# skeskinen/bert.cpp

Measured on AMD Instinct MI355X. Metric: sentences/sec (seq_len=128), higher is better.
Workload: dtype f16; 1 GPU; all-MiniLM-L6-v2 f16, batch=256 seq_len=128; per_gpu_batch=256, global_batch=256, seq_len=128, weights=f16, parallelism=dp1 (replicated weights, sharded sentences)

## Files before the change

### bert.cpp_amd/csrc/layer_tail.hip

```cpp
#include "tile_stream.h"

namespace bert_hip {

namespace {

constexpr int LT_TILE = 16384;
#ifndef LT_ABLATE
#define LT_ABLATE 0
#endif
#ifndef LT_UPRIO
#define LT_UPRIO 1
#endif
#ifndef LT_GELU_BATCH
#define LT_GELU_BATCH 0
#endif
#ifndef LT_DMA_SPLIT
#define LT_DMA_SPLIT 1
#endif
#ifndef LT_DPRIO
#define LT_DPRIO 0
#endif

typedef float f32x2 __attribute__((ext_vector_type(2)));

// ... 46 lines not shown
    asm volatile("ds_read_b64 %0, %1 offset:%2" : "=v"(v) : "v"(addr), "n"(OFF) : "memory");
    return v;
}
template <int OFF>
__device__ __forceinline__ f32x4 lds_read_f32x4_h(unsigned addr) {
    f32x4 v;
    asm volatile("ds_read_b128 %0, %1 offset:%2" : "=v"(v) : "v"(addr), "n"(OFF) : "memory");
    return v;
}
template <int OFF>
__device__ __forceinline__ f16x8 frag_read(unsigned addr) {
    if (LT_ABLATE & 4) { f16x8 z = (f16x8)(_Float16)0.f; asm volatile("" : "+v"(z) : "v"(addr)); return z; }
    return lds_read_b128_u<OFF>(addr);
}

__device__ __forceinline__ void dma_m0(unsigned lds) {
    if (LT_ABLATE & 1) return;
    asm volatile("s_mov_b32 m0, %0" : : "s"(lds) : "memory");
}
template <int PIECE>
__device__ __forceinline__ void dma_piece(const char *gbase, unsigned voff) {
    if (LT_ABLATE & 1) return;
    asm volatile("global_load_lds_dwordx4 %0, %1 offset:%2" : : "v"(voff), "s"(gbase - PIECE * 1024), "n"(PIECE * 1024) : "memory");
}

__device__ __forceinline__ f32x16 mfma16(const f16x8 &a, const f16x8 &b, const f32x16 &c) {
    if (LT_ABLATE & 8) { f32x16 r = c; asm volatile("" : "+v"(r[0]) : "v"(a), "v"(b)); return r; }
    return __builtin_amdgcn_mfma_f32_32x32x16_f16(a, b, c, 0, 0, 0);
}

}

template <int NT, int WT, bool RAGGED = false>
__device__ __forceinline__ void layer_tail_body(const TailArgs &a, char *smem, const int tok0, const int rows, const int tid) {
    constexpr bool Q4 = WT != GW_F16;
    constexpr int VMQ = Q4 ? 63 : 0;
    constexpr int H = 128 * NT, NBH = 2 * NT, NB = 4 * NT, NQ = 8 * NT, NYH = 4 * NT;
    constexpr int P = NT * NT;
    constexpr int NG = NT;
    constexpr int LAGT = NT + NG;
    const int I = a.I, NC = I / 64;
    const int lane = tid & 63;
    const int wave = __builtin_amdgcn_readfirstlane(tid >> 6);
    const int t = wave & 3, role = wave >> 2;
    const int l31 = lane & 31, hi = lane >> 5;
    const int tok_w = tok0 + t * 32;
    const int row_l = RAGGED ? tok0 + min(t * 32 + l31, rows - 1) : tok_w + l31;

    char *ringU = smem;
    char *ringD = smem + 3 * LT_TILE;
    char *G = smem + 6 * LT_TILE;
    float *ST = (float *)(G + 32768);
    float *cbo = ST + 8 * 64;
    float *cg1 = cbo + H, *cbe1 = cg1 + H, *cb2 = cbe1 + H, *cg2 = cb2 + H, *cbe2 = cg2 + H, *cb1 = cbe2 + H;

    {
        constexpr int NPB = 4;
        const float *const src[6] = {a.bo, a.g1, a.be1, a.b2, a.g2, a.be2};
        float pv[6];
        f32x4 bq[NPB];
#pragma unroll
        for (int k = 0; k < 6; ++k) pv[k] = tid < H ? src[k][tid] : 0.f;
#pragma unroll
        for (int k = 0; k < NPB; ++k) {
            const int i4 = (k * 512 + tid) * 4;
            bq[k] = i4 < I ? *(const f32x4 *)(a.b1 + i4) : f32x4{0.f, 0.f, 0.f, 0.f};
        }
// ... 87 lines not shown
    auto dma_proj = [&](int n3, int kt, unsigned tile) __attribute__((always_inline)) {
        if constexpr (Q4) q4_request_rows(a.wo_qs, a.wo_sc, n3 * (H / 64) + kt);
        else dma128(wo + (size_t)n3 * 128 * H + kt * 64, offH, H * 2, tile);
    };
    auto dma_up = [&](int c, int j, unsigned offU, unsigned tile) __attribute__((always_inline)) {
        if constexpr (Q4) q4_request_up(c, j);
        else dma_up_f16(c, j, offU, tile);
    };

    const unsigned aR = lds_addr(ringU) + (unsigned)off64(l31, hi);
    const unsigned aUp = lds_addr(ringU) + (unsigned)(l31 * 256 + ((hi ^ (l31 & 15)) << 4));

    int slot = 0;
    [[maybe_unused]] int tl = 1;
    [[maybe_unused]] const bool tlU = tid == 0, tlD = tid == 256;
    LT_STAMP(tlU, 0);
    auto pre_close = [&]() __attribute__((always_inline)) { LT_STAMP_FINE(tlU, 128 + tl); LT_STAMP_FINE(tlD, 256 + tl); };
    auto next_slot = [&]() __attribute__((always_inline)) { slot = slot == 2 ? 0 : slot + 1; LT_STAMP(tlU, tl); ++tl; };
    auto slot_plus2 = [&]() __attribute__((always_inline)) { return slot == 0 ? 2 : slot - 1; };
    [[maybe_unused]] auto slot_plus1 = [&]() __attribute__((always_inline)) { return slot == 2 ? 0 : slot + 1; };
    using PLAIN = std::false_type; using PERMUTED = std::true_type;

    auto proj_request = [&](int p, int s) __attribute__((always_inline)) {
        const int n3 = p / NT, q = p % NT;
        if (role == 0) dma_proj(n3, 2 * q, ldsU + s * LT_TILE);
        else dma_proj(n3, 2 * q + 1, ldsD + s * LT_TILE);
    };
    proj_request(0, 0);
    q4_expand_rows(PLAIN{}, role ? ringD : ringU);
    proj_request(1, 1);
    LT_STAMP(tlU, 384);
    asm volatile("s_waitcnt vmcnt(0) lgkmcnt(0)\n\ts_barrier" ::: "memory");
    LT_STAMP(tlU, 385);
#pragma unroll
    for (int b = 0; b < NBH; ++b)
#pragma unroll
        for (int gq = 0; gq < 4; ++gq) {
            const f32x4 bv = *(const f32x4 *)(cbo + (b >> 1) * 128 + role * 64 + (b & 1) * 32 + 8 * gq + 4 * hi);
#pragma unroll
            for (int e = 0; e < 4; ++e) accp[b][4 * gq + e] = (float)xv[b][gq][e] + bv[e];
        }
#pragma unroll
    for (int b = 0; b < NBH; ++b) asm volatile("" : "+v"(accp[b]));
    __builtin_amdgcn_s_waitcnt(0xc07f);
    static_for<P>([&](auto p_tag) __attribute__((always_inline)) {
        constexpr int p = decltype(p_tag)::value, n3 = p / NT, q = p % NT, p2 = p + 2;
        const unsigned bA = aR + (unsigned)(slot * LT_TILE + role * 8192), bB = bA + 3 * LT_TILE;
        f16x8 Fa[4], Fb[4];
        auto rd = [&](unsigned base, int g2, f16x8 (&F)[4]) __attribute__((always_inline)) {
            const unsigned a0 = base ^ (unsigned)((2 * g2) << 5), a1 = base ^ (unsigned)((2 * g2 + 1) << 5);
            F[0] = frag_read<0>(a0); F[1] = frag_read<4096>(a0);
            F[2] = frag_read<0>(a1); F[3] = frag_read<4096>(a1);
        };
        auto mm = [&](f16x8 (&F)[4], int ks) __attribute__((always_inline)) {
            accp[n3 * 2 + 0] = mfma16(F[0], bf[ks], accp[n3 * 2 + 0]);
            accp[n3 * 2 + 1] = mfma16(F[1], bf[ks], accp[n3 * 2 + 1]);
            accp[n3 * 2 + 0] = mfma16(F[2], bf[ks + 1], accp[n3 * 2 + 0]);
            accp[n3 * 2 + 1] = mfma16(F[3], bf[ks + 1], accp[n3 * 2 + 1]);
        };
        auto q4_turn = [&]() __attribute__((always_inline)) {
            if constexpr (p + 1 < P) q4_expand_rows(PLAIN{}, (role ? ringD : ringU) + slot_plus1() * LT_TILE);
            else if (role == 1) q4_expand_up(ringU + slot_plus1() * LT_TILE);
            const int s2 = slot_plus2();
            if constexpr (p2 < P) proj_request(p2, s2);
            else if (role == 1) dma_up(0, p2 - P, up_offset(), ldsU + s2 * LT_TILE);
        };
// ... 362 lines not shown
                    request(std::integral_constant<bool, up>{}, FF{}, c * NT + d + LAGT + 2, 0);
                    if constexpr (pend_dn) q4_expand_rows(PERMUTED{}, ringD + slot_plus1() * LT_TILE);
                    request(FF{}, std::integral_constant<bool, dn>{}, 0, c * NT + d + 2);
                    __builtin_amdgcn_sched_barrier(0);
                }
                rd(std::integral_constant<int, 0>{}, Fa, ga);
                rd(std::integral_constant<int, 1>{}, Fb, gb);
                wait_group(N5{}, Fa, ga);
                mm(Fa, ga);
                rd(std::integral_constant<int, 2>{}, Fa, ga);
                if constexpr (!Q4) {
                    if constexpr (LT_DMA_SPLIT) request(std::integral_constant<bool, up>{}, FF{}, c * NT + d + LAGT + 2, 0);
                    else request(std::integral_constant<bool, up>{}, std::integral_constant<bool, dn>{}, c * NT + d + LAGT + 2, c * NT + d + 2);
                }
                wait_group(N5{}, Fb, gb);
                mm(Fb, gb);
                rd(std::integral_constant<int, 3>{}, Fb, gb);
                if constexpr (!Q4 && LT_DMA_SPLIT) request(FF{}, std::integral_constant<bool, dn>{}, 0, c * NT + d + 2);
                wait_group(N5{}, Fa, ga);
                mm(Fa, ga);
                wait_group(N0{}, Fb, gb);
                mm(Fb, gb);
                pre_close();
                close_interval<Q4 ? 63 : (up ? 4 : 0) + (dn ? 4 : 0)>();
                next_slot();
            });
        };
        static_assert(LAGT == 2 * NT, "the request schedule below assumes D runs two chunks behind");
        (void)NUP;
        for (int c = 0; c + 3 < NC; ++c) d_chunk(std::integral_constant<int, NT>{}, FF{}, TT{}, c);
        d_chunk(std::integral_constant<int, NT - 2>{}, FF{}, TT{}, NC - 3);
        d_chunk(std::integral_constant<int, 0>{}, FF{}, FF{}, NC - 2);
        d_chunk(std::integral_constant<int, 0>{}, TT{}, FF{}, NC - 1);

        {
            char *S = smem + t * (64 * H);
            int lane = (int)__builtin_amdgcn_mbcnt_hi(~0u, __builtin_amdgcn_mbcnt_lo(~0u, 0u));
            asm volatile("" : "+v"(lane));
            const int hi = lane >> 5;
            {
                const char *const xu = ringU + t * (NYH * 1024) + lane * 16;
#pragma unroll
                for (int n3 = 0; n3 < NT; ++n3) {
                    f16x8 yu[4];
#pragma unroll
                    for (int m = 0; m < 4; ++m) yu[m] = *(const f16x8 *)(xu + (4 * n3 + m) * 1024);
#pragma unroll
                    for (int m = 0; m < 4; ++m)
#pragma unroll
                        for (int e = 0; e < 8; ++e) acc2[4 * n3 + (m >> 1)][8 * (m & 1) + e] += (float)yu[m][e];
                    asm volatile("" ::: "memory");
                }
            }
            asm volatile("s_waitcnt lgkmcnt(0)\n\ts_barrier" ::: "memory");
            float s1 = 0.f, s2 = 0.f;
#pragma unroll
            for (int n = 0; n < NB; ++n)
#pragma unroll
                for (int r = 0; r < 16; ++r) { s1 += acc2[n][r]; s2 = __builtin_fmaf(acc2[n][r], acc2[n][r], s2); }
            s1 += __shfl_xor(s1, 32);
            s2 += __shfl_xor(s2, 32);
            float rstd, nmr;
            layernorm_scale(s1, s2, 1.0f / H, rstd, nmr);
#pragma unroll
            for (int n = 0; n < NB; ++n) {
                f32x4 gv[4], bv[4];
// ... 94 lines not shown
```

### bert.cpp_amd/csrc/model_kernel.hip

```cpp
#define BERT_HIP_PHASES_ONLY
#include "qkv_attention2.hip"
#include "layer_tail.hip"
#undef BERT_HIP_PHASES_ONLY
#include "pool_normalize.h"

namespace bert_hip {

#ifdef BERT_HIP_MODEL_TIMELINE
static __device__ unsigned long long g_tl_model[1024 * 32];
#define MK_STAMP(i) do { const int mk_i = (i); if (threadIdx.x == 0 && mk_i < 32) g_tl_model[(blockIdx.x & 1023) * 32 + mk_i] = __builtin_amdgcn_s_memrealtime(); } while (0)
#else
#define MK_STAMP(i) do { } while (0)
#endif

namespace {

constexpr int MODEL_MAX_LAYERS = 12;

struct ModelLayerArgs {
    const half_t *wqkv, *wo, *w1p, *w2p;
    const float *bqkv, *bo, *g1, *be1, *b1, *b2, *g2, *be2;
};
struct ModelArgs {
    half_t *x, *ctx;
    const int32_t *cu;
    const int2 *groups;
    const int *n_groups;
    int n_layer, n_head, n_sent, I, slot_mask;
    float *pooled;
    int *status;
    int max_len;
    ModelLayerArgs layer[MODEL_MAX_LAYERS];
};

}

template <int NT, bool RAGGED>
__global__ __launch_bounds__(512, 2) void model_kernel(ModelArgs m) {
    extern __shared__ __attribute__((aligned(16))) char smem[];
    const int window = (int)blockIdx.x;
    int tok0 = window * 128, rows = 128, first = window, count = 1;
    if constexpr (RAGGED) {
        if (m.groups) {
            if (m.n_groups && window >= *m.n_groups) return;
            const int2 g = m.groups[window];
            first = g.x; count = g.y;
        }
        if (count <= 0 || first >= m.n_sent) return;
        tok0 = m.cu[first];
        rows = min(m.cu[first + count] - tok0, 128);
    }
    const int wave_index = __builtin_amdgcn_readfirstlane((int)threadIdx.x >> 6);
    auto thread_id = [&]() __attribute__((always_inline)) {
        int ln = (int)__builtin_amdgcn_mbcnt_hi(~0u, __builtin_amdgcn_mbcnt_lo(~0u, 0u)), w = wave_index;
        asm volatile("" : "+v"(ln), "+s"(w));
        return w * 64 + ln;
    };
    MK_STAMP(0);
    const int n_layer = rows > 0 ? m.n_layer : 0;
    for (int l = 0; l < n_layer; ++l) {
        const ModelLayerArgs &L = m.layer[l];
        int tid = thread_id();
        {
            Qkv2Args q;
            q.x = m.x; q.w = L.wqkv; q.qs = nullptr; q.sc = nullptr; q.bias = L.bqkv; q.cu = m.cu; q.groups = RAGGED ? m.groups : nullptr; q.n_groups = nullptr;
            q.out = m.ctx; q.n_head = m.n_head; q.n_sent = m.n_sent; q.spw = 1; q.slot_mask = m.slot_mask;
            qkv_attention2_body<2 * NT, NT, GW_F16>(q, smem, window, tid);
        }
        __builtin_amdgcn_fence(__ATOMIC_RELEASE, "workgroup");
        asm volatile("s_waitcnt vmcnt(0) lgkmcnt(0)\n\ts_barrier" ::: "memory");
        __builtin_amdgcn_fence(__ATOMIC_ACQUIRE, "workgroup");
        MK_STAMP(1 + 2 * l);
        tid = thread_id();
        {
            TailArgs t;
            t.ctx = m.ctx; t.x = m.x; t.wo = L.wo; t.w1p = L.w1p; t.w2p = L.w2p;
            t.wo_qs = t.w1_qs = t.w2_qs = nullptr; t.wo_sc = t.w1_sc = t.w2_sc = nullptr;
            t.bo = L.bo; t.g1 = L.g1; t.be1 = L.be1; t.b1 = L.b1; t.b2 = L.b2; t.g2 = L.g2; t.be2 = L.be2; t.out = m.x; t.I = m.I;
            layer_tail_body<NT, GW_F16, RAGGED>(t, smem, tok0, rows, tid);
        }
        __builtin_amdgcn_fence(__ATOMIC_RELEASE, "workgroup");
        asm volatile("s_waitcnt vmcnt(0) lgkmcnt(0)\n\ts_barrier" ::: "memory");
        __builtin_amdgcn_fence(__ATOMIC_ACQUIRE, "workgroup");
        MK_STAMP(2 + 2 * l);
    }
    if (m.pooled) {
        const int tid = thread_id();
        for (int j = 0; j < count; ++j) {
            const int b = first + j, t0 = m.cu[b];
            int n = m.cu[b + 1] - t0;
            if (!RAGGED && (t0 != tok0 || n != 128)) n = -1;
            pool_normalize_sentence(m.x, t0, n, b, 128 * NT, m.max_len, m.status, m.pooled, (float *)smem, tid, tid < 256);
            __syncthreads();
        }
    }
    MK_STAMP(1 + 2 * n_layer);
}

bool model_kernel_supported(const GemmWeight &Wqkv, const GemmWeight &Wo, const GemmWeight &W1, const GemmWeight &W2, int n_layer,
                            int n_head, int d_head, int max_len) {
    const int H = n_head * d_head;
    return n_layer <= MODEL_MAX_LAYERS && (H == 256 || H == 384) && max_len >= 1 && max_len <= 128 &&
           Wqkv.type == GW_F16 && Wo.type == GW_F16 && qkv_attention2_supported(Wqkv, n_head, d_head, max_len) && layer_tail_supported(Wo, W1, W2);
}

void launch_model_kernel(const ModelLayerWeights *layers, int n_layer, half_t *x, half_t *ctx, const int32_t *cu_seqlens, int n_sentences,
                         int n_tokens, const int2 *groups, int n_groups, const int *n_groups_dev, int n_head, float *pooled, int max_len,
                         int *status, int slots, hipStream_t stream) {
    ModelArgs m;
    m.pooled = pooled; m.status = status; m.max_len = max_len;
    m.x = x; m.ctx = ctx; m.cu = cu_seqlens; m.groups = groups; m.n_groups = n_groups_dev;
    m.n_layer = n_layer; m.n_head = n_head; m.n_sent = n_sentences; m.I = layers[0].W1->N; m.slot_mask = slots - 1;
    for (int l = 0; l < n_layer; ++l) {
        const ModelLayerWeights &s = layers[l];
        ModelLayerArgs &d = m.layer[l];
        d.wqkv = s.Wqkv->w16; d.wo = s.Wo->w16; d.w1p = s.W1->w16p; d.w2p = s.W2->w16p;
        d.bqkv = s.bqkv; d.bo = s.bo; d.g1 = s.g1; d.be1 = s.be1; d.b1 = s.b1; d.b2 = s.b2; d.g2 = s.g2; d.be2 = s.be2;
    }
    const int H = layers[0].W1->K, KT = H / 64, GB = KT / 2;
    const size_t lds_q = (size_t)3 * GB * Q2_TILE + 2 * (2 * Q2_WIN * 64 + 32 * Q2_VT_LD * 2) + (size_t)2 * H * sizeof(float);
    const size_t lds = std::max(lds_q, layer_tail_lds(H, m.I));
    const bool full = (long long)n_sentences * 128 == n_tokens;
    const int grid = full || !groups ? n_sentences : n_groups;
    static DeviceFlags configured[4];
    auto go = [&](auto kernel, int which) {
        configure_once(configured[which], [&] { (void)hipFuncSetAttribute((const void *)kernel, hipFuncAttributeMaxDynamicSharedMemorySize, 160 * 1024); });
        BERT_LAUNCH(kernel, dim3(grid), dim3(512), lds, stream, m);
#ifdef BERT_HIP_MODEL_TIMELINE
        static int shots = 0;
        if (grid >= 256 && shots++ == 30) {
            (void)hipDeviceSynchronize();
            static unsigned long long h[1024 * 32];
            (void)hipMemcpyFromSymbol(h, HIP_SYMBOL(g_tl_model), sizeof(h));
            const int nw = grid < 1024 ? grid : 1024, ns = 2 + 2 * n_layer;
            unsigned long long t0 = ~0ull;
            for (int w = 0; w < nw; ++w) t0 = h[w * 32] < t0 ? h[w * 32] : t0;
            fprintf(stderr, "model_kernel timeline, %d workgroups (us after the first workgroup's start: min mean max):\n", nw);
            for (int i = 0; i < ns; ++i) {
                double lo = 1e30, hi = 0, sum = 0;
                for (int w = 0; w < nw; ++w) { const double v = (double)(h[w * 32 + i] - t0) * 0.01; lo = v < lo ? v : lo; hi = v > hi ? v : hi; sum += v; }
                fprintf(stderr, "  stamp %2d: %8.2f %8.2f %8.2f\n", i, lo, sum / nw, hi);
            }
            fprintf(stderr, "  mean phase durations (window, tail) per layer:");
            for (int l = 0; l < n_layer; ++l) {
                double a = 0, b = 0;
                for (int w = 0; w < nw; ++w) { a += (double)(h[w * 32 + 1 + 2 * l] - h[w * 32 + 2 * l]) * 0.01; b += (double)(h[w * 32 + 2 + 2 * l] - h[w * 32 + 1 + 2 * l]) * 0.01; }
                fprintf(stderr, " (%.1f, %.1f)", a / nw, b / nw);
            }
            fprintf(stderr, "\n  mean end per XCD:");
            for (int x = 0; x < 8; ++x) {
                double e = 0; int c = 0;
                for (int w = x; w < nw; w += 8) { e += (double)(h[w * 32 + ns - 1] - t0) * 0.01; ++c; }
                fprintf(stderr, " %.1f", e / c);
            }
            fprintf(stderr, "\n  mean end per eighth of the grid:");
            for (int x = 0; x < 8; ++x) {
                double e = 0; int c = 0;
                for (int w = x * nw / 8; w < (x + 1) * nw / 8; ++w) { e += (double)(h[w * 32 + ns - 1] - t0) * 0.01; ++c; }
                fprintf(stderr, " %.1f", e / c);
            }
            double pl = 0;
            for (int w = 0; w < nw; ++w) pl += (double)(h[w * 32 + 1 + 2 * n_layer] - h[w * 32 + 2 * n_layer]) * 0.01;
            fprintf(stderr, "; pooling %.2f\n", pl / nw);
        }
#endif
    };
    if (full) { if (H == 256) go(model_kernel<2, false>, 0); else go(model_kernel<3, false>, 1); }
    else { if (H == 256) go(model_kernel<2, true>, 2); else go(model_kernel<3, true>, 3); }
}

}
```

### bert.cpp_amd/csrc/qkv_attention2.hip

```cpp
#include "tile_stream.h"

#ifndef Q2_PM
#define Q2_PM 3
#endif
#ifndef Q2_PRIO
#define Q2_PRIO 0
#endif

namespace bert_hip {

namespace {

constexpr int Q2_WIN = 128;
constexpr int Q2_TILE = 12288;
constexpr int Q2_VT_LD = Q2_WIN + 4;

struct Qkv2Args {
    const half_t *x;
    const half_t *w;
    const uint4 *qs;
    const void *sc;
    const float *bias;
    const int32_t *cu;
    const int2 *groups;
// ... 15 lines not shown
__device__ __forceinline__ void q2_wait6(f16x8 (&f)[2][3]) {
    asm volatile("s_waitcnt lgkmcnt(6)"
                 : "+v"(f[0][0]), "+v"(f[0][1]), "+v"(f[0][2]), "+v"(f[1][0]), "+v"(f[1][1]), "+v"(f[1][2]) : : "memory");
}
template <int VM>
__device__ __forceinline__ void q2_slab_barrier(f16x8 (&f)[2][3]) {
    asm volatile("s_waitcnt vmcnt(%6) lgkmcnt(0)\n\ts_barrier"
                 : "+v"(f[0][0]), "+v"(f[0][1]), "+v"(f[0][2]), "+v"(f[1][0]), "+v"(f[1][1]), "+v"(f[1][2]) : "n"(VM) : "memory");
}
__device__ __forceinline__ void q2_wait14(f16x8 (&f)[2][3]) {
    asm volatile("s_waitcnt lgkmcnt(14)"
                 : "+v"(f[0][0]), "+v"(f[0][1]), "+v"(f[0][2]), "+v"(f[1][0]), "+v"(f[1][1]), "+v"(f[1][2]) : : "memory");
}
__device__ __forceinline__ void q2_wait0_bias(f16x8 (&f)[2][3], f32x4 (&bq)[4], f32x4 (&bk)[4]) {
    asm volatile("s_waitcnt lgkmcnt(0)"
                 : "+v"(f[0][0]), "+v"(f[0][1]), "+v"(f[0][2]), "+v"(f[1][0]), "+v"(f[1][1]), "+v"(f[1][2]),
                   "+v"(bq[0]), "+v"(bq[1]), "+v"(bq[2]), "+v"(bq[3]), "+v"(bk[0]), "+v"(bk[1]), "+v"(bk[2]), "+v"(bk[3]) : : "memory");
}
template <int OFF>
__device__ __forceinline__ f32x4 q2_read_f32x4(unsigned addr) {
    f32x4 v;
    asm volatile("ds_read_b128 %0, %1 offset:%2" : "=v"(v) : "v"(addr), "n"(OFF));
    return v;
}
__device__ __forceinline__ void q2_take(float &bv) { asm volatile("" : "+v"(bv)); }
template <int VM>
__device__ __forceinline__ void q2_head_barrier() {
    asm volatile("s_waitcnt vmcnt(%0) lgkmcnt(0)\n\ts_barrier" : : "n"(VM) : "memory");
}

}

template <int KT, int GB, int WT>
__device__ __forceinline__ void qkv_attention2_body(const Qkv2Args &a, char *smem, const int window, const int tid) {
    constexpr bool Q4 = WT != GW_F16;
    constexpr int H = 64 * KT, NBAR = KT / GB, SLAB = GB * Q2_TILE, PPS = 3 * GB;
    static_assert(KT == 2 * GB && NBAR == 2, "");
    constexpr int QKV_BYTES = 2 * Q2_WIN * 64 + 32 * Q2_VT_LD * 2;
    char *RING = smem;
    char *QKV = smem + 3 * SLAB;
    float *BS = (float *)(QKV + 2 * QKV_BYTES);

    const int lane = tid & 63;
    const int wave = __builtin_amdgcn_readfirstlane(tid >> 6);
    const int l31 = lane & 31, hi = lane >> 5;
    const int blk = wave & 3;
    const int n_head = a.n_head;
    TL_STAMP_AT(tid == 256, 120);
    TL_REALTIME_AT(tid == 256, 121);
    TL_STAMP_AT(tid == 0, 250);
    TL_REALTIME_AT(tid == 0, 251);

    const int wp = blk;
    const unsigned loff = (unsigned)(((wp * 8 + (lane >> 3)) * H + (((lane & 7) ^ (((wp & 1) << 2) | ((lane >> 4) & 3))) * 8)) * 2);
    auto dma_piece = [&](const char *hbase, auto j_tag, int dslot, auto i_tag) __attribute__((always_inline)) {
        constexpr int i = decltype(i_tag)::value, j = decltype(j_tag)::value, t = i / 3, rb = i % 3;
        const char *src = hbase + ((size_t)rb * H * H + (size_t)(j * GB + t) * 64) * 2;
        __builtin_amdgcn_global_load_lds(AS_GLOBAL(src + loff), AS_LDS(RING + dslot * SLAB + t * Q2_TILE + rb * 4096 + wp * 1024), 16, 0, 0);
    };
    const char *const wbase = (const char *)a.w;
    if constexpr (!Q4) {
        if (wave >= 4) static_for<PPS>([&](auto i) __attribute__((always_inline)) { dma_piece(wbase, std::integral_constant<int, 0>{}, 0, i); });
    }

    int first, count;
    if (a.groups) {
        if (a.n_groups && window >= *a.n_groups) {
            asm volatile("s_waitcnt vmcnt(0)" ::: "memory");
            return;
        }
        const int2 g = a.groups[window];
        first = g.x; count = g.y;
    }
    else { first = window * a.spw; count = min(a.spw, a.n_sent - first); }
    if (count <= 0) {
        asm volatile("s_waitcnt vmcnt(0)" ::: "memory");
        return;
    }
    const int slot = blk * 32 + l31;
    int gtok = -1, k0 = 0, k1 = 0;
    {
        const int place = a.groups ? 128 : 128 / a.spw;
        int off = 0;
        for (int j = 0; j < count; ++j) {
            const int t0 = a.cu[first + j], n = min(a.cu[first + j + 1] - t0, place);
            if (slot >= off && slot < off + n) { gtok = t0 + slot - off; k0 = off; k1 = off + n; }
            off = (off + n + a.slot_mask) & ~a.slot_mask;
        }
    }

    if (wave >= 4) {
        f16x8 bf[4 * KT];
        {
            const int gt = gtok >= 0 ? gtok : a.cu[first];
            const half_t *xr = a.x + (size_t)gt * H + 8 * hi;
#pragma unroll
            for (int ks = 0; ks < 4 * KT; ++ks) asm volatile("global_load_dwordx4 %0, %1, off" : "=v"(bf[ks]) : "v"(xr + 16 * ks));
        }
        if constexpr (!Q4) static_for<PPS>([&](auto i) __attribute__((always_inline)) { dma_piece(wbase, std::integral_constant<int, NBAR - 1>{}, 1, i); });

        constexpr int NRAW = GB;
        [[maybe_unused]] RawBlock raw[NRAW];
        auto q4_image_of_lane = [&]() __attribute__((always_inline)) {
            int ln = (int)__builtin_amdgcn_mbcnt_hi(~0u, __builtin_amdgcn_mbcnt_lo(~0u, 0u));
            asm volatile("" : "+v"(ln));
            return (ln >> 1) * 128 + (((4 * (ln & 1)) ^ ((ln >> 2) & 7)) << 4);
        };
        auto q4_rb = [&](int hq, int j, int i) __attribute__((always_inline)) { return (blk + i + 2 * hq + j) & 3; };
        auto q4_request = [&](int hq, int j, int i) __attribute__((always_inline)) {
            if constexpr (Q4) {
                const int rb = q4_rb(hq, j, i);
                if (rb == 3) return;
                const int sbase = ((rb * (H / 128) + (hq >> 2)) * (H / 64) + j * GB + i) * 256 + (hq & 3) * 64;
                raw[i] = q4_load_block<WT>(a.qs + sbase, WT == GW_Q4_0 ? (const void *)((const unsigned short *)a.sc + sbase) : (const void *)((const unsigned *)a.sc + sbase), (size_t)lane);
            }
        };
        auto q4_expand = [&](int hq, int j, int dslot, int i) __attribute__((always_inline)) {
            if constexpr (Q4) {
                const int rb = q4_rb(hq, j, i);
                if (rb == 3) return;
                char *const base = RING + dslot * SLAB + i * Q2_TILE + rb * 4096;
                const int q4_image = q4_image_of_lane();
                q4_expand_block<WT, false>(raw[i], [&](int k) __attribute__((always_inline)) { return base + (q4_image ^ (k << 4)); });
            }
        };
        if constexpr (Q4) {
            RawBlock first[2][NRAW];
#pragma unroll
            for (int j = 0; j < 2; ++j)
#pragma unroll
// ... 8 lines not shown
                    raw[i] = first[j][i];
                    q4_expand(0, j, j, i);
                }
        }
        const unsigned aX0 = lds_addr(RING) + off64(l31, hi);
        unsigned aS[4];
        int rslot = 0;
        auto set_slot = [&]() __attribute__((always_inline)) {
#pragma unroll
            for (int kk = 0; kk < 4; ++kk) aS[kk] = (aX0 ^ (unsigned)(kk << 5)) + (unsigned)rslot * SLAB;
        };
        set_slot();
        f16x8 F[2][2][3];
        f32x16 acc[3];
        auto read_half = [&](auto par_tag, auto tt_tag, auto half_tag) __attribute__((always_inline)) {
            constexpr int par = decltype(par_tag)::value, tt = decltype(tt_tag)::value, half = decltype(half_tag)::value;
#pragma unroll
            for (int i = 0; i < 2; ++i) {
                F[par][i][0] = q2_read_b128<tt * Q2_TILE>(aS[2 * half + i]);
                F[par][i][1] = q2_read_b128<tt * Q2_TILE + 4096>(aS[2 * half + i]);
                F[par][i][2] = q2_read_b128<tt * Q2_TILE + 8192>(aS[2 * half + i]);
            }
        };
        [[maybe_unused]] const bool tl_sel = tid == 256;
        TL_STAMP_AT(tl_sel, 0);
        asm volatile("s_waitcnt vmcnt(%0) lgkmcnt(0)\n\ts_barrier" : : "n"(Q4 ? 0 : PPS) : "memory");
#pragma unroll
        for (int ks = 0; ks < 4 * KT; ++ks) asm volatile("" : "+v"(bf[ks]));
        if constexpr (Q4) {
#pragma unroll
            for (int i = 0; i < NRAW; ++i) q4_request(min(1, n_head - 1), 0, i);
        }
        TL_STAMP_AT(tl_sel, 1);
        read_half(std::integral_constant<int, 0>{}, std::integral_constant<int, 0>{}, std::integral_constant<int, 0>{});

        const unsigned aBias = lds_addr(BS) + 16 * hi;
        for (int h = 0; h < n_head; ++h) {
            char *QS = QKV + (h & 1) * QKV_BYTES, *KS = QS + Q2_WIN * 64;
            half_t *VT = (half_t *)(KS + Q2_WIN * 64);
            float bv;
            if constexpr (Q4) bv = a.bias[2 * H + h * 32 + l31];
            else asm volatile("global_load_dword %0, %1, off" : "=v"(bv) : "v"(a.bias + 2 * H + h * 32 + l31));
            f32x4 bq[4], bk[4];
            const char *const hnext = wbase + (size_t)min(h + 1, n_head - 1) * 32 * H * 2;
#pragma unroll
            for (int m = 0; m < 3; ++m)
#pragma unroll
                for (int r = 0; r < 16; ++r) acc[m][r] = 0.f;
            constexpr int LT0 = 2 * KT - 2, LT1 = 2 * KT - 1;
            auto pieces = [&](auto hh_tag, auto m_tag) __attribute__((always_inline)) {
                constexpr int hh = decltype(hh_tag)::value, m = decltype(m_tag)::value, hs = hh % (2 * GB);
                constexpr int i0 = (3 * hs + 1) / 2, i1 = (3 * (hs + 1) + 1) / 2;
                const int dslot = (hh == 2 * GB - 1) ? (rslot == 2 ? 0 : rslot + 1) : (rslot == 0 ? 2 : rslot - 1);
                if constexpr (Q4) {
                    constexpr int j = (hh >> 1) / GB;
                    if constexpr (m == 1) {
                        if constexpr (hs < GB) { if (h + 1 < n_head) q4_expand(h + 1, j, dslot, hs); }
                        else q4_request(min(j == 0 ? h + 1 : h + 2, n_head - 1), j ^ 1, hs - GB);
                    }
                } else {
                if constexpr (m == 1) dma_piece(hnext, std::integral_constant<int, (hh >> 1) / GB>{}, dslot, std::integral_constant<int, i0>{});
                if constexpr (m == 4 && i1 - i0 == 2) dma_piece(hnext, std::integral_constant<int, (hh >> 1) / GB>{}, dslot, std::integral_constant<int, i0 + 1>{});
                }
            };
            auto mma = [&](auto par_tag, auto i_tag, auto rb_tag, auto ks_tag) __attribute__((always_inline)) {
                constexpr int par = decltype(par_tag)::value, i = decltype(i_tag)::value, rb = decltype(rb_tag)::value, ks = decltype(ks_tag)::value;
// ... 54 lines not shown
                    }
#pragma unroll
                    for (int gg = 0; gg < 4; ++gg) {
                        f16x4 ov;
#pragma unroll
                        for (int e = 0; e < 4; ++e) ov[e] = (_Float16)(acc[2][4 * gg + e] + bv);
                        *(f16x4 *)(VT + l31 * Q2_VT_LD + blk * 32 + 8 * gg + 4 * hi) = ov;
                    }
                }
            });
            if (h < 8) TL_STAMP_AT(tl_sel, 2 + 6 * h + 4);
            q2_head_barrier<Q4 ? 63 : PPS>();
            if (h < 8) TL_STAMP_AT(tl_sel, 2 + 6 * h + 5);
            rslot = rslot == 2 ? 0 : rslot + 1;
            set_slot();
            read_half(std::integral_constant<int, 0>{}, std::integral_constant<int, 0>{}, std::integral_constant<int, 0>{});
        }
        TL_STAMP_AT(tl_sel, 60);
        asm volatile("s_waitcnt vmcnt(0)" ::: "memory");
    } else {
        unsigned need = 0, inner = 0;
#pragma unroll
        for (int kt = 0; kt < 4; ++kt) {
            const bool nd = gtok >= 0 && k0 < 32 * kt + 32 && k1 > 32 * kt;
            const bool in = gtok < 0 || (k0 <= 32 * kt && k1 >= 32 * kt + 32);
            if (__any(nd)) need |= 1u << kt;
            if (__all(in)) inner |= 1u << kt;
        }
        need = __builtin_amdgcn_readfirstlane(need);
        inner = __builtin_amdgcn_readfirstlane(inner);
        const unsigned klen = (unsigned)(k1 - k0);
        const int kbase = 4 * hi - k0;
        const float sc = 1.44269504088896340736f / __builtin_sqrtf(32.0f);
        for (int i = tid; i < 2 * H; i += 256) BS[i] = a.bias[i];
        asm volatile("s_waitcnt vmcnt(0) lgkmcnt(0)\n\ts_barrier" ::: "memory");

        if constexpr (Q2_PRIO > 0) __builtin_amdgcn_s_setprio(Q2_PRIO);
        [[maybe_unused]] const bool tl_sel = tid == 0;
        auto attend = [&](int hh, auto wb_tag, auto fast_tag, int tb) __attribute__((always_inline)) {
            constexpr bool WB = decltype(wb_tag)::value, FAST = decltype(fast_tag)::value;
            const char *QS = QKV + (hh & 1) * QKV_BYTES, *KS = QS + Q2_WIN * 64;
            const half_t *VT = (const half_t *)(KS + Q2_WIN * 64);
            f32x16 s[4];
            f16x8 qf[2];
#pragma unroll
            for (int kk = 0; kk < 2; ++kk) qf[kk] = *(const f16x8 *)(QS + q2_off32(slot, kk * 2 + hi));
            float mx = -INFINITY;
            int kb = kbase;
            unsigned kl = klen;
            if constexpr (!FAST) asm volatile("" : "+v"(kb), "+v"(kl));
#pragma unroll
            for (int kt = 0; kt < 4; ++kt) {
                if (FAST || (need & (1u << kt))) {
#pragma unroll
                    for (int r = 0; r < 16; ++r) s[kt][r] = 0.f;
#pragma unroll
                    for (int kk = 0; kk < 2; ++kk) {
                        const f16x8 kf = *(const f16x8 *)(KS + q2_off32(kt * 32 + l31, kk * 2 + hi));
                        s[kt] = __builtin_amdgcn_mfma_f32_32x32x16_f16(kf, qf[kk], s[kt], 0, 0, 0);
                    }
                    if (FAST || (inner & (1u << kt))) {
#pragma unroll
                        for (int r = 0; r < 16; ++r) mx = fmaxf(mx, s[kt][r]);
                    } else {
#pragma unroll
                        for (int r = 0; r < 16; ++r) {
                            const bool ok = (unsigned)(kt * 32 + (r & 3) + 8 * (r >> 2) + kb) < kl;
                            const float v = ok ? s[kt][r] : -INFINITY;
// ... 24 lines not shown
                        const f16x8 pf = softmax_p8(s[kt][8 * st], s[kt][8 * st + 1], s[kt][8 * st + 2], s[kt][8 * st + 3], s[kt][8 * st + 4],
                                                    s[kt][8 * st + 5], s[kt][8 * st + 6], s[kt][8 * st + 7], sc, mx, psum);
                        const int key0 = kt * 32 + 16 * st + 4 * hi;
                        const half_t *vr = VT + l31 * Q2_VT_LD + key0;
                        const f16x4 v0 = *(const f16x4 *)vr, v1 = *(const f16x4 *)(vr + 8);
                        f16x8 vf;
#pragma unroll
                        for (int e = 0; e < 4; ++e) { vf[e] = v0[e]; vf[4 + e] = v1[e]; }
                        o = __builtin_amdgcn_mfma_f32_32x32x16_f16(vf, pf, o, 0, 0, 0);
                    }
                }
                if constexpr (WB) {
                    if (kt + 4 == Q2_PM) {
                        if (tb < 8) TL_STAMP_AT(tl_sel, 128 + 6 * tb + 1);
                        asm volatile("s_barrier" ::: "memory");
                        if (tb < 8) TL_STAMP_AT(tl_sel, 128 + 6 * tb + 2);
                    }
                }
            }
            psum = xor32_sum(psum);
            if (gtok >= 0) {
                const float inv = 1.0f / psum;
                half_t *op = a.out + (size_t)gtok * H + hh * 32;
#pragma unroll
                for (int gq = 0; gq < 4; ++gq) {
                    f16x4 ov;
#pragma unroll
                    for (int e = 0; e < 4; ++e) ov[e] = (_Float16)rounded_f32(o[4 * gq + e] * inv);
                    *(f16x4 *)(op + 8 * gq + 4 * hi) = ov;
                }
            }
        };
        const bool fast = need == 0xFu && inner == 0xFu;
        asm volatile("s_barrier" ::: "memory");
        asm volatile("s_barrier" ::: "memory");
        for (int h = 1; h < n_head; ++h) {
            if (h < 8) TL_STAMP_AT(tl_sel, 128 + 6 * h);
            if (fast) attend(h - 1, std::true_type{}, std::true_type{}, h);
            else attend(h - 1, std::true_type{}, std::false_type{}, h);
            if (h < 8) TL_STAMP_AT(tl_sel, 128 + 6 * h + 5);
            asm volatile("s_barrier" ::: "memory");
        }
        TL_STAMP_AT(tl_sel, 190);
        if (fast) attend(n_head - 1, std::false_type{}, std::true_type{}, 0);
        else attend(n_head - 1, std::false_type{}, std::false_type{}, 0);
        TL_STAMP_AT(tl_sel, 192);
        TL_STAMP_AT(tl_sel, 252);
        TL_REALTIME_AT(tl_sel, 253);
    }
}

template <int KT, int GB, int WT>
__global__ __launch_bounds__(512, 2) void qkv_attention2_kernel(Qkv2Args a) {
    extern __shared__ __attribute__((aligned(16))) char smem[];
    qkv_attention2_body<KT, GB, WT>(a, smem, (int)blockIdx.x, (int)threadIdx.x);
}

#ifndef BERT_HIP_PHASES_ONLY
constexpr int BW_THREADS = 512;

template <int SLOT>
__global__ __launch_bounds__(BW_THREADS) void build_windows_kernel(const int32_t *__restrict__ cu, int B, int2 *__restrict__ windows,
                                                                   int *__restrict__ n_windows) {
    constexpr int BW_STATES = 128 / SLOT + 1;
    __shared__ unsigned char exit_state[BW_THREADS][BW_STATES];
    __shared__ int closes[BW_THREADS][BW_STATES];
    __shared__ int opened[BW_THREADS][BW_STATES];
    __shared__ int entry_fill[BW_THREADS], entry_first[BW_THREADS], entry_index[BW_THREADS];
    const int t = threadIdx.x, per = (B + BW_THREADS - 1) / BW_THREADS, n_blocks = per ? (B + per - 1) / per : 0;
    const int b0 = min(B, t * per), b1 = min(B, b0 + per);

    int fill[BW_STATES], n_closed[BW_STATES], first[BW_STATES];
#pragma unroll
    for (int e = 0; e < BW_STATES; ++e) { fill[e] = e * SLOT; n_closed[e] = 0; first[e] = -1; }
    for (int b = b0; b < b1; ++b) {
        const int n = cu[b + 1] - cu[b];
// ... 91 lines not shown
```

### bert.cpp_amd/csrc/tile_stream.h

```cpp
#pragma once
#include "kernels.h"

#include <cstdio>
#include <type_traits>
#include <utility>

namespace bert_hip {

typedef _Float16 f16x4 __attribute__((ext_vector_type(4)));
typedef _Float16 f16x8 __attribute__((ext_vector_type(8)));
typedef float f32x4 __attribute__((ext_vector_type(4)));
typedef float f32x16 __attribute__((ext_vector_type(16)));

template <int... I, class F>
__device__ __forceinline__ void static_for_impl(std::integer_sequence<int, I...>, F &&f) {
    (f(std::integral_constant<int, I>{}), ...);
}
template <int N, class F>
__device__ __forceinline__ void static_for(F &&f) { static_for_impl(std::make_integer_sequence<int, N>{}, f); }

#define AS_GLOBAL(p) ((const __attribute__((address_space(1))) void *)(p))
#define AS_LDS(p) ((__attribute__((address_space(3))) void *)(p))


#ifdef BERT_HIP_TIMELINE
static __device__ unsigned long long g_timeline[1024 * 256];
#define TL_STAMP(i) do { const int tl_i = (i); if (threadIdx.x == 0 && tl_i < 256) g_timeline[(blockIdx.x & 1023) * 256 + tl_i] = __builtin_readcyclecounter(); } while (0)
#define TL_STAMP_AT(sel, i) do { const int tl_i = (i); if ((sel) && tl_i < 256) g_timeline[(blockIdx.x & 1023) * 256 + tl_i] = __builtin_readcyclecounter(); } while (0)
#define TL_REALTIME_AT(sel, i) do { const int tl_i = (i); if ((sel) && tl_i < 256) g_timeline[(blockIdx.x & 1023) * 256 + tl_i] = __builtin_amdgcn_s_memrealtime(); } while (0)
#define TL_DUMP(cond, nstamps) do {                                                                          \
    static int tl_shots = 0;                                                                                  \
    if ((cond) && tl_shots++ == 20) {                                                                         \
        (void)hipDeviceSynchronize();                                                                         \
        static unsigned long long tl_h[1024 * 256];                                                           \
        (void)hipMemcpyFromSymbol(tl_h, HIP_SYMBOL(g_timeline), sizeof(tl_h));                                \
        const int tl_n = (nstamps) < 256 ? (nstamps) : 256;                                                   \
        for (int b : {0, 1, 100, 255}) {                                                                      \
            fprintf(stderr, "timeline wg %3d:", b);                                                           \
            for (int i = 1; i < tl_n; ++i) fprintf(stderr, " %llu", tl_h[b * 256 + i] - tl_h[b * 256 + i - 1]); \
            fprintf(stderr, "  total %llu\n", tl_h[b * 256 + tl_n - 1] - tl_h[b * 256]);                      \
        }                                                                                                     \
    }                                                                                                         \
} while (0)
#define TL_DUMP_RAW(cond, nstamps) do {                                                                      \
    static int tl_shots = 0;                                                                                  \
    if ((cond) && tl_shots++ == 20) {                                                                         \
        (void)hipDeviceSynchronize();                                                                         \
        static unsigned long long tl_h[1024 * 256];                                                           \
        (void)hipMemcpyFromSymbol(tl_h, HIP_SYMBOL(g_timeline), sizeof(tl_h));                                \
        for (int b : {0, 100}) {                                                                              \
            fprintf(stderr, "rawtimeline wg %3d:", b);                                                        \
            for (int i = 0; i < (nstamps); ++i)                                                               \
                fprintf(stderr, " %lld", tl_h[b * 256 + i] ? (long long)(tl_h[b * 256 + i] - tl_h[b * 256]) : -1LL); \
            fprintf(stderr, "\n");                                                                            \
        }                                                                                                     \
    }                                                                                                         \
// ... 179 lines not shown
```

Measured before the change: 319,700 sentences/s.

## Keep layer output in LDS across layers and reload QKV activations from LDS

In the fused per-window model kernel, layers after the first read the QKV input activations straight from the previous layer tail's LDS staging area instead of reloading them from global memory. The weight DMA is deferred until after those LDS reads, and the end-of-layer full barrier is dropped except after the last layer. The bias preload now uses an async global-to-LDS load, and the cu offsets go through a scalar-address-space pointer. Phase clocks are also added for the model timeline build, which is off by default. The risk is LDS aliasing hazards if the tail's staging layout or barrier ordering doesn't exactly match what the QKV stage assumes.

```diff
diff --git a/bert.cpp_amd/csrc/layer_tail.hip b/bert.cpp_amd/csrc/layer_tail.hip
--- a/bert.cpp_amd/csrc/layer_tail.hip
+++ b/bert.cpp_amd/csrc/layer_tail.hip
@@ -102,7 +102,8 @@
 }
 
 template <int NT, int WT, bool RAGGED = false>
-__device__ __forceinline__ void layer_tail_body(const TailArgs &a, char *smem, const int tok0, const int rows, const int tid) {
+__device__ __forceinline__ void layer_tail_body(const TailArgs &a, char *smem, const int tok0, const int rows, const int tid,
+                                                [[maybe_unused]] unsigned long long *clk = nullptr) {
     constexpr bool Q4 = WT != GW_F16;
     constexpr int VMQ = Q4 ? 63 : 0;
     constexpr int H = 128 * NT, NBH = 2 * NT, NB = 4 * NT, NQ = 8 * NT, NYH = 4 * NT;
@@ -256,6 +257,7 @@
     LT_STAMP(tlU, 384);
     asm volatile("s_waitcnt vmcnt(0) lgkmcnt(0)\n\ts_barrier" ::: "memory");
     LT_STAMP(tlU, 385);
+    PH_CLOCK(clk, 4);
 #pragma unroll
     for (int b = 0; b < NBH; ++b)
 #pragma unroll
@@ -684,6 +686,7 @@
         d_chunk(std::integral_constant<int, NT - 2>{}, FF{}, TT{}, NC - 3);
         d_chunk(std::integral_constant<int, 0>{}, FF{}, FF{}, NC - 2);
         d_chunk(std::integral_constant<int, 0>{}, TT{}, FF{}, NC - 1);
+        PH_CLOCK(clk, 5);
 
         {
             char *S = smem + t * (64 * H);
diff --git a/bert.cpp_amd/csrc/model_kernel.hip b/bert.cpp_amd/csrc/model_kernel.hip
--- a/bert.cpp_amd/csrc/model_kernel.hip
+++ b/bert.cpp_amd/csrc/model_kernel.hip
@@ -6,11 +6,20 @@
 
 namespace bert_hip {
 
+constexpr int MK_PER_LAYER = 7;
+#ifndef MK_X_LDS
+#define MK_X_LDS 1
+#endif
 #ifdef BERT_HIP_MODEL_TIMELINE
-static __device__ unsigned long long g_tl_model[1024 * 32];
-#define MK_STAMP(i) do { const int mk_i = (i); if (threadIdx.x == 0 && mk_i < 32) g_tl_model[(blockIdx.x & 1023) * 32 + mk_i] = __builtin_amdgcn_s_memrealtime(); } while (0)
+constexpr int MK_SLOTS = 128;
+static __device__ unsigned long long g_tl_model[1024 * MK_SLOTS];
+#define MK_CLOCK(v) ((v) = __builtin_amdgcn_s_memrealtime())
+#define MK_WRITE(tid0, i, v) do { if (threadIdx.x == (tid0)) g_tl_model[(blockIdx.x & 1023) * MK_SLOTS + (i)] = (v); } while (0)
+#define MK_CLOCKS(c) (c)
 #else
-#define MK_STAMP(i) do { } while (0)
+#define MK_CLOCKS(c) nullptr
+#define MK_CLOCK(v) do { } while (0)
+#define MK_WRITE(tid0, i, v) do { } while (0)
 #endif
 
 namespace {
@@ -56,33 +65,47 @@
         asm volatile("" : "+v"(ln), "+s"(w));
         return w * 64 + ln;
     };
-    MK_STAMP(0);
+    [[maybe_unused]] unsigned long long clk[MK_PER_LAYER] = {};
+    MK_CLOCK(clk[0]);
+    MK_WRITE(0, 0, clk[0]);
     const int n_layer = rows > 0 ? m.n_layer : 0;
     for (int l = 0; l < n_layer; ++l) {
         const ModelLayerArgs &L = m.layer[l];
         int tid = thread_id();
+        MK_CLOCK(clk[0]);
         {
             Qkv2Args q;
             q.x = m.x; q.w = L.wqkv; q.qs = nullptr; q.sc = nullptr; q.bias = L.bqkv; q.cu = m.cu; q.groups = RAGGED ? m.groups : nullptr; q.n_groups = nullptr;
             q.out = m.ctx; q.n_head = m.n_head; q.n_sent = m.n_sent; q.spw = 1; q.slot_mask = m.slot_mask;
-            qkv_attention2_body<2 * NT, NT, GW_F16>(q, smem, window, tid);
+            qkv_attention2_body<2 * NT, NT, GW_F16>(q, smem, window, tid, MK_X_LDS && l > 0, MK_CLOCKS(clk));
         }
         __builtin_amdgcn_fence(__ATOMIC_RELEASE, "workgroup");
         asm volatile("s_waitcnt vmcnt(0) lgkmcnt(0)\n\ts_barrier" ::: "memory");
         __builtin_amdgcn_fence(__ATOMIC_ACQUIRE, "workgroup");
-        MK_STAMP(1 + 2 * l);
+        MK_CLOCK(clk[3]);
+        {
+            [[maybe_unused]] const int b = 1 + MK_PER_LAYER * l;
+            if (l > 0) { MK_WRITE(0, b - 3, clk[4]); MK_WRITE(256, b - 2, clk[5]); MK_WRITE(0, b - 1, clk[6]); }
+            MK_WRITE(0, b, clk[0]); MK_WRITE(256, b + 1, clk[1]); MK_WRITE(0, b + 2, clk[2]); MK_WRITE(0, b + 3, clk[3]);
+        }
         tid = thread_id();
         {
             TailArgs t;
             t.ctx = m.ctx; t.x = m.x; t.wo = L.wo; t.w1p = L.w1p; t.w2p = L.w2p;
             t.wo_qs = t.w1_qs = t.w2_qs = nullptr; t.wo_sc = t.w1_sc = t.w2_sc = nullptr;
             t.bo = L.bo; t.g1 = L.g1; t.be1 = L.be1; t.b1 = L.b1; t.b2 = L.b2; t.g2 = L.g2; t.be2 = L.be2; t.out = m.x; t.I = m.I;
-            layer_tail_body<NT, GW_F16, RAGGED>(t, smem, tok0, rows, tid);
+            layer_tail_body<NT, GW_F16, RAGGED>(t, smem, tok0, rows, tid, MK_CLOCKS(clk));
         }
-        __builtin_amdgcn_fence(__ATOMIC_RELEASE, "workgroup");
-        asm volatile("s_waitcnt vmcnt(0) lgkmcnt(0)\n\ts_barrier" ::: "memory");
-        __builtin_amdgcn_fence(__ATOMIC_ACQUIRE, "workgroup");
-        MK_STAMP(2 + 2 * l);
+        if (!MK_X_LDS || l + 1 == n_layer) {
+            __builtin_amdgcn_fence(__ATOMIC_RELEASE, "workgroup");
+            asm volatile("s_waitcnt vmcnt(0) lgkmcnt(0)\n\ts_barrier" ::: "memory");
+            __builtin_amdgcn_fence(__ATOMIC_ACQUIRE, "workgroup");
+        }
+        MK_CLOCK(clk[6]);
+    }
+    if (n_layer > 0) {
+        [[maybe_unused]] const int b = 1 + MK_PER_LAYER * n_layer;
+        MK_WRITE(0, b - 3, clk[4]); MK_WRITE(256, b - 2, clk[5]); MK_WRITE(0, b - 1, clk[6]);
     }
     if (m.pooled) {
         const int tid = thread_id();
@@ -94,7 +117,8 @@
             __syncthreads();
         }
     }
-    MK_STAMP(1 + 2 * n_layer);
+    MK_CLOCK(clk[0]);
+    MK_WRITE(0, 1 + MK_PER_LAYER * n_layer, clk[0]);
 }
 
 bool model_kernel_supported(const GemmWeight &Wqkv, const GemmWeight &Wo, const GemmWeight &W1, const GemmWeight &W2, int n_layer,
@@ -130,38 +154,34 @@
         static int shots = 0;
         if (grid >= 256 && shots++ == 30) {
             (void)hipDeviceSynchronize();
-            static unsigned long long h[1024 * 32];
+            static unsigned long long h[1024 * MK_SLOTS];
             (void)hipMemcpyFromSymbol(h, HIP_SYMBOL(g_tl_model), sizeof(h));
-            const int nw = grid < 1024 ? grid : 1024, ns = 2 + 2 * n_layer;
+            const int nw = grid < 1024 ? grid : 1024, last = 1 + MK_PER_LAYER * n_layer;
             unsigned long long t0 = ~0ull;
-            for (int w = 0; w < nw; ++w) t0 = h[w * 32] < t0 ? h[w * 32] : t0;
-            fprintf(stderr, "model_kernel timeline, %d workgroups (us after the first workgroup's start: min mean max):\n", nw);
-            for (int i = 0; i < ns; ++i) {
-                double lo = 1e30, hi = 0, sum = 0;
-                for (int w = 0; w < nw; ++w) { const double v = (double)(h[w * 32 + i] - t0) * 0.01; lo = v < lo ? v : lo; hi = v > hi ? v : hi; sum += v; }
-                fprintf(stderr, "  stamp %2d: %8.2f %8.2f %8.2f\n", i, lo, sum / nw, hi);
+            for (int w = 0; w < nw; ++w) t0 = h[w * MK_SLOTS] < t0 ? h[w * MK_SLOTS] : t0;
+            auto mean = [&](int i, int j) {
+                double a = 0;
+                for (int w = 0; w < nw; ++w) a += (double)(long long)(h[w * MK_SLOTS + j] - h[w * MK_SLOTS + i]) * 0.01;
+                return a / nw;
+            };
+            fprintf(stderr, "model_kernel phase clock, %d workgroups, mean us per layer:\n"
+                            "  layer  w.prologue  w.steady  w.last-head+edge  t.prologue  t.steady  t.epilogue+edge | layer\n", nw);
+            double sum[6] = {};
+            for (int l = 0; l < n_layer; ++l) {
+                const int b = 1 + MK_PER_LAYER * l;
+                double d[6];
+                for (int k = 0; k < 6; ++k) { d[k] = mean(b + k, b + k + 1); sum[k] += d[k]; }
+                fprintf(stderr, "  %5d  %10.2f  %8.2f  %16.2f  %10.2f  %8.2f  %15.2f | %6.2f\n", l, d[0], d[1], d[2], d[3], d[4], d[5],
+                        mean(b, b + 6));
             }
-            fprintf(stderr, "  mean phase durations (window, tail) per layer:");
-            for (int l = 0; l < n_layer; ++l) {
-                double a = 0, b = 0;
-                for (int w = 0; w < nw; ++w) { a += (double)(h[w * 32 + 1 + 2 * l] - h[w * 32 + 2 * l]) * 0.01; b += (double)(h[w * 32 + 2 + 2 * l] - h[w * 32 + 1 + 2 * l]) * 0.01; }
-                fprintf(stderr, " (%.1f, %.1f)", a / nw, b / nw);
+            fprintf(stderr, "  all    %10.2f  %8.2f  %16.2f  %10.2f  %8.2f  %15.2f | %6.2f\n", sum[0], sum[1], sum[2], sum[3], sum[4], sum[5],
+                    mean(0, last));
+            double lo = 1e30, hi = 0, e = 0;
+            for (int w = 0; w < nw; ++w) {
+                const double v = (double)(h[w * MK_SLOTS + last] - t0) * 0.01;
+                lo = v < lo ? v : lo; hi = v > hi ? v : hi; e += v;
             }
-            fprintf(stderr, "\n  mean end per XCD:");
-            for (int x = 0; x < 8; ++x) {
-                double e = 0; int c = 0;
-                for (int w = x; w < nw; w += 8) { e += (double)(h[w * 32 + ns - 1] - t0) * 0.01; ++c; }
-                fprintf(stderr, " %.1f", e / c);
-            }
-            fprintf(stderr, "\n  mean end per eighth of the grid:");
-            for (int x = 0; x < 8; ++x) {
-                double e = 0; int c = 0;
-                for (int w = x * nw / 8; w < (x + 1) * nw / 8; ++w) { e += (double)(h[w * 32 + ns - 1] - t0) * 0.01; ++c; }
-                fprintf(stderr, " %.1f", e / c);
-            }
-            double pl = 0;
-            for (int w = 0; w < nw; ++w) pl += (double)(h[w * 32 + 1 + 2 * n_layer] - h[w * 32 + 2 * n_layer]) * 0.01;
-            fprintf(stderr, "; pooling %.2f\n", pl / nw);
+            fprintf(stderr, "  pooled (us after the first start): min %.1f mean %.1f max %.1f; pooling %.2f\n", lo, e / nw, hi, mean(last - 1, last));
         }
 #endif
     };
diff --git a/bert.cpp_amd/csrc/qkv_attention2.hip b/bert.cpp_amd/csrc/qkv_attention2.hip
--- a/bert.cpp_amd/csrc/qkv_attention2.hip
+++ b/bert.cpp_amd/csrc/qkv_attention2.hip
@@ -71,7 +71,8 @@
 }
 
 template <int KT, int GB, int WT>
-__device__ __forceinline__ void qkv_attention2_body(const Qkv2Args &a, char *smem, const int window, const int tid) {
+__device__ __forceinline__ void qkv_attention2_body(const Qkv2Args &a, char *smem, const int window, const int tid, const bool x_lds = false,
+                                                    [[maybe_unused]] unsigned long long *clk = nullptr) {
     constexpr bool Q4 = WT != GW_F16;
     constexpr int H = 64 * KT, NBAR = KT / GB, SLAB = GB * Q2_TILE, PPS = 3 * GB;
     static_assert(KT == 2 * GB && NBAR == 2, "");
@@ -99,9 +100,13 @@
     };
     const char *const wbase = (const char *)a.w;
     if constexpr (!Q4) {
-        if (wave >= 4) static_for<PPS>([&](auto i) __attribute__((always_inline)) { dma_piece(wbase, std::integral_constant<int, 0>{}, 0, i); });
-    }
-
+        if (wave >= 4 && !x_lds) static_for<PPS>([&](auto i) __attribute__((always_inline)) { dma_piece(wbase, std::integral_constant<int, 0>{}, 0, i); });
+    }
+
+    const int32_t *cu_p = a.cu;
+    asm volatile("" : "+s"(cu_p));
+    const __attribute__((address_space(4))) int32_t *const cu_s = (const __attribute__((address_space(4))) int32_t *)cu_p;
+    auto cu = [&](int i) __attribute__((always_inline)) { return a.groups ? a.cu[i] : cu_s[i]; };
     int first, count;
     if (a.groups) {
         if (a.n_groups && window >= *a.n_groups) {
@@ -122,7 +127,7 @@
         const int place = a.groups ? 128 : 128 / a.spw;
         int off = 0;
         for (int j = 0; j < count; ++j) {
-            const int t0 = a.cu[first + j], n = min(a.cu[first + j + 1] - t0, place);
+            const int t0 = cu(first + j), n = min(cu(first + j + 1) - t0, place);
             if (slot >= off && slot < off + n) { gtok = t0 + slot - off; k0 = off; k1 = off + n; }
             off = (off + n + a.slot_mask) & ~a.slot_mask;
         }
@@ -131,10 +136,26 @@
     if (wave >= 4) {
         f16x8 bf[4 * KT];
         {
-            const int gt = gtok >= 0 ? gtok : a.cu[first];
-            const half_t *xr = a.x + (size_t)gt * H + 8 * hi;
-#pragma unroll
-            for (int ks = 0; ks < 4 * KT; ++ks) asm volatile("global_load_dwordx4 %0, %1, off" : "=v"(bf[ks]) : "v"(xr + 16 * ks));
+            const int gt = gtok >= 0 ? gtok : cu(first);
+            if (x_lds) {
+                const int r = gt - cu(first);
+                const char *S = smem + (r >> 5) * (64 * H) + 8 * hi;
+                const int o = (r & 31) * 16;
+#pragma unroll
+                for (int ks = 0; ks < 4 * KT; ++ks) {
+                    const int p = (o + 32 * ks) & 1023;
+                    const f16x4 lo = *(const f16x4 *)(S + ks * 1024 + p), up = *(const f16x4 *)(S + ks * 1024 + (p ^ 512));
+#pragma unroll
+                    for (int e = 0; e < 4; ++e) { bf[ks][e] = lo[e]; bf[ks][4 + e] = up[e]; }
+                }
+                __builtin_amdgcn_s_waitcnt(0xc07f);
+                asm volatile("s_barrier" ::: "memory");
+                if constexpr (!Q4) static_for<PPS>([&](auto i) __attribute__((always_inline)) { dma_piece(wbase, std::integral_constant<int, 0>{}, 0, i); });
+            } else {
+                const half_t *xr = a.x + (size_t)gt * H + 8 * hi;
+#pragma unroll
+                for (int ks = 0; ks < 4 * KT; ++ks) asm volatile("global_load_dwordx4 %0, %1, off" : "=v"(bf[ks]) : "v"(xr + 16 * ks));
+            }
         }
         if constexpr (!Q4) static_for<PPS>([&](auto i) __attribute__((always_inline)) { dma_piece(wbase, std::integral_constant<int, NBAR - 1>{}, 1, i); });
 
@@ -209,6 +230,7 @@
             for (int i = 0; i < NRAW; ++i) q4_request(min(1, n_head - 1), 0, i);
         }
         TL_STAMP_AT(tl_sel, 1);
+        PH_CLOCK(clk, 1);
         read_half(std::integral_constant<int, 0>{}, std::integral_constant<int, 0>{}, std::integral_constant<int, 0>{});
 
         const unsigned aBias = lds_addr(BS) + 16 * hi;
@@ -329,8 +351,10 @@
         const unsigned klen = (unsigned)(k1 - k0);
         const int kbase = 4 * hi - k0;
         const float sc = 1.44269504088896340736f / __builtin_sqrtf(32.0f);
-        for (int i = tid; i < 2 * H; i += 256) BS[i] = a.bias[i];
-        asm volatile("s_waitcnt vmcnt(0) lgkmcnt(0)\n\ts_barrier" ::: "memory");
+        if (x_lds) asm volatile("s_barrier" ::: "memory");
+        asm volatile("s_barrier" ::: "memory");
+        if (blk < GB)
+            __builtin_amdgcn_global_load_lds(AS_GLOBAL(a.bias + blk * 256 + lane * 4), AS_LDS((char *)BS + blk * 1024), 16, 0, 0);
 
         if constexpr (Q2_PRIO > 0) __builtin_amdgcn_s_setprio(Q2_PRIO);
         [[maybe_unused]] const bool tl_sel = tid == 0;
@@ -421,6 +445,7 @@
             }
         };
         const bool fast = need == 0xFu && inner == 0xFu;
+        __builtin_amdgcn_s_waitcnt(0x0f70);
         asm volatile("s_barrier" ::: "memory");
         asm volatile("s_barrier" ::: "memory");
         for (int h = 1; h < n_head; ++h) {
@@ -431,6 +456,7 @@
             asm volatile("s_barrier" ::: "memory");
         }
         TL_STAMP_AT(tl_sel, 190);
+        PH_CLOCK(clk, 2);
         if (fast) attend(n_head - 1, std::false_type{}, std::true_type{}, 0);
         else attend(n_head - 1, std::false_type{}, std::false_type{}, 0);
         TL_STAMP_AT(tl_sel, 192);
diff --git a/bert.cpp_amd/csrc/tile_stream.h b/bert.cpp_amd/csrc/tile_stream.h
--- a/bert.cpp_amd/csrc/tile_stream.h
+++ b/bert.cpp_amd/csrc/tile_stream.h
@@ -22,6 +22,12 @@
 #define AS_GLOBAL(p) ((const __attribute__((address_space(1))) void *)(p))
 #define AS_LDS(p) ((__attribute__((address_space(3))) void *)(p))
 
+
+#ifdef BERT_HIP_MODEL_TIMELINE
+#define PH_CLOCK(clk, k) do { if (clk) (clk)[k] = __builtin_amdgcn_s_memrealtime(); } while (0)
+#else
+#define PH_CLOCK(clk, k) do { } while (0)
+#endif
 
 #ifdef BERT_HIP_TIMELINE
 static __device__ unsigned long long g_timeline[1024 * 256];
```

Result: faster. 323,100 sentences/s, median of 6 (+1.1%).
